# yeeus/GCI

Measured on AMD Instinct MI355X. Metric: aligned Gbases/s through filter+depth pipeline (CHM13, 40x HiFi), higher is better.
Workload: dtype int32

## Files before the change

### gci_amd/csrc/api_ctx.hip

```cpp
#include "gci_ctx.hpp"
#include <stdlib.h>
#include <vector>

int gci_fail(gci_ctx* c, hipError_t e, const char* what)
{
    if (c) c->err = std::string(what) + ": " + hipGetErrorString(e);
    return GCI_E_HIP;
}

int gci_ensure(gci_ctx* ctx, DevBuf& b, size_t bytes)
{
    if (bytes <= b.cap) return GCI_OK;
    if (b.p) { HIPCHK(hipStreamSynchronize(ctx->stream)); HIPCHK(gci_dfree(b.p)); b.p = nullptr; b.cap = 0; }
    size_t want = bytes + bytes / 4 + 256;
    HIPCHK(gci_dmalloc(ctx->device, &b.p, want));
    b.cap = want;
    return GCI_OK;
}

int gci_upload_small(gci_ctx* ctx, void* d_dst, const void* h_src, size_t bytes)
{
    HIPCHK(hipStreamSynchronize(ctx->stream));
    if (bytes > ctx->h_pinned_cap) {
        if (ctx->h_pinned) HIPCHK(hipHostFree(ctx->h_pinned));
        ctx->h_pinned = nullptr;
        ctx->h_pinned_cap = 0;
        size_t want = bytes * 2 + 4096;
        HIPCHK(hipHostMalloc(&ctx->h_pinned, want, hipHostMallocDefault));
        ctx->h_pinned_cap = want;
    }
    memcpy(ctx->h_pinned, h_src, bytes);
    HIPCHK(hipMemcpyAsync(d_dst, ctx->h_pinned, bytes, hipMemcpyHostToDevice, ctx->stream));
    return GCI_OK;
}

extern "C" int gci_abi_version(void) { return GCI_ABI_VERSION; }

extern "C" int gci_ctx_create(int device, void* stream, int own_stream, gci_ctx** out)
{
    if (!out) return GCI_E_INVALID;
    gci_ctx* ctx = new (std::nothrow) gci_ctx();
    if (!ctx) return GCI_E_NOMEM;
    ctx->device = device;
    { const char* fd = getenv("GCI_FORCE_DENSE"); if (fd && fd[0] == '1') ctx->sparse_max = -1; }
    { const char* m = getenv("GCI_JOIN"); ctx->join_mode = m && m[0] == 'c' ? 1 : m && m[0] == 'p' ? 2 : 0; }
    hipError_t e = hipSetDevice(device);
    if (e != hipSuccess) { delete ctx; return GCI_E_HIP; }
    if (!own_stream) { ctx->stream = (hipStream_t)stream; }
    else {
        e = hipStreamCreateWithFlags(&ctx->stream, hipStreamNonBlocking);
        if (e != hipSuccess) { delete ctx; return GCI_E_HIP; }
        ctx->own_stream = true;
    }
    {
        uint32_t lut[TEXT_LUT];
        gci_text_lut_host(lut);
        if (gci_dmalloc(device, &ctx->text_lut.p, sizeof lut) != hipSuccess ||
            hipMemcpy(ctx->text_lut.p, lut, sizeof lut, hipMemcpyHostToDevice) != hipSuccess) {
            gci_ctx_destroy(ctx);
            return GCI_E_HIP;
        }
        ctx->text_lut.cap = sizeof lut;
    }
    *out = ctx;
    return GCI_OK;
}

extern "C" int gci_ctx_destroy(gci_ctx* ctx)
{
    if (!ctx) return GCI_OK;
    (void)hipSetDevice(ctx->device);
    (void)hipStreamSynchronize(ctx->stream);
    DevBuf* bufs[] = {&ctx->d_len, &ctx->d_off, &ctx->d_tile_first, &ctx->tile_cd, &ctx->tile_carry, &ctx->dense_flag, &ctx->dense_list, &ctx->evp_items, &ctx->evp_hist, &ctx->evp_blk, &ctx->d_tile_valid,
                      &ctx->evt_off, &ctx->events, &ctx->blk_a, &ctx->blk_b, &ctx->tile_sum, &ctx->tile_u32,
                      &ctx->tile_u64, &ctx->blk_u64, &ctx->join_table, &ctx->join_last, &ctx->join_hq, &ctx->part_a, &ctx->part_b, &ctx->part_hist, &ctx->part_blk, &ctx->conflict_table, &ctx->win,
                      &ctx->win_tile_first, &ctx->text_lut, &ctx->long_items, &ctx->pg_scan, &ctx->pg_first, &ctx->route_tab, &ctx->deflate_nruns, &ctx->deflate_runs, &ctx->deflate_tab, &ctx->dgz_tiles, &ctx->build_nruns, &ctx->build_runs, &ctx->join_bucket, &ctx->tail_gaps, &ctx->tail_sums, &ctx->class_sums, &ctx->crc_tabs, &ctx->inflate_sym, &ctx->inflate_nsym, &ctx->inflate_wstatus, &ctx->inflate_lists, &ctx->inflate_prof, &ctx->inflate_next, &ctx->inflate_sym2, &ctx->inflate_lists2,
                      &ctx->bg_tile_cnt, &ctx->bg_tile_off, &ctx->bg_blk, &ctx->bg_wtab, &ctx->bg_blk_bytes, &ctx->bg_blk_off, &ctx->bg_blk2, &ctx->hist_chunk_first,
                      &ctx->cover_rec, &ctx->cover_chunk};
    for (DevBuf* b : bufs) if (b->p) (void)gci_dfree(b->p);
    for (DevBuf& b : ctx->paf_pool) if (b.p) (void)gci_dfree(b.p);
    if (ctx->h_pinned) (void)hipHostFree(ctx->h_pinned);
    for (auto* v : {&ctx->prof_live, &ctx->prof_free}) for (auto& e : *v) { (void)hipEventDestroy(e.a); (void)hipEventDestroy(e.b); }
    if (ctx->inflate_stream2) { (void)hipStreamSynchronize(ctx->inflate_stream2); (void)hipStreamDestroy(ctx->inflate_stream2); }
    if (ctx->inflate_ev_in) (void)hipEventDestroy(ctx->inflate_ev_in);
    if (ctx->inflate_ev_out) (void)hipEventDestroy(ctx->inflate_ev_out);
    if (ctx->own_stream) (void)hipStreamDestroy(ctx->stream);
    delete ctx;
    return GCI_OK;
}

extern "C" int gci_sync(gci_ctx* ctx)
{
    if (!ctx) return GCI_E_INVALID;
    HIPCHK(hipStreamSynchronize(ctx->stream));
    return GCI_OK;
}

extern "C" const char* gci_strerror(int s)
{
    switch (s) {
    case GCI_OK: return "ok";
    case GCI_E_INVALID: return "invalid argument";
    case GCI_E_HIP: return "HIP runtime error";
    case GCI_E_NO_NM: return "record without NM tag (reference raises KeyError, GCI.py:163)";
    case GCI_E_ZERO_DIV: return "zero denominator (reference raises ZeroDivisionError, GCI.py:165/292)";
    case GCI_E_BAD_NM_TYPE: return "NM tag is not an integer";
    case GCI_E_NO_END: return "record has no CIGAR: reference_end is None";
    case GCI_E_MALFORMED: return "malformed BAM record";
    case GCI_E_CAPACITY: return "output capacity exceeded";
    case GCI_E_NOMEM: return "out of memory";
    case GCI_E_NO_LAYOUT: return "gci_layout_set() not called";
    default: return "unknown status";
    }
}

extern "C" const char* gci_last_error(gci_ctx* ctx) { return ctx ? ctx->err.c_str() : ""; }

static const char* const PROF_NAMES[GCI_PROF_COUNT] = {
    "k_bam_filter", "k_join_insert", "k_join_fold", "k_evt_count+scatter", "k_scan2", "k_tile_build", "k_gap_mask",
    "k_max2", "k_issue_scan", "k_text_count", "k_text_write", "k_depth_sum", "memset", "k_tile_pass1", "k_tile_dense",
    "k_part1+k_part2 (radix partition of the join)", "k_join_part", "k_pg_measure+scans+k_pg_first (record pages: sizes)", "k_pg_write (record pages)"};

extern "C" int gci_profile_enable(gci_ctx* ctx, int mask)
{
    if (!ctx) return GCI_E_INVALID;
    ctx->prof_mask = mask;
    return GCI_OK;
}

extern "C" int gci_profile_read(gci_ctx* ctx, int kernel_id, double* total_ms, uint64_t* launches, int reset)
{
    if (!ctx || kernel_id < 0 || kernel_id >= GCI_PROF_COUNT) return GCI_E_INVALID;
    HIPCHK(hipStreamSynchronize(ctx->stream));
    for (auto& e : ctx->prof_live) {
        float ms = 0.f;
        if (hipEventElapsedTime(&ms, e.a, e.b) == hipSuccess) { ctx->prof_ms[e.id] += ms; ctx->prof_n[e.id]++; }
        ctx->prof_free.push_back(e);
    }
    ctx->prof_live.clear();
    if (total_ms) *total_ms = ctx->prof_ms[kernel_id];
    if (launches) *launches = ctx->prof_n[kernel_id];
    if (reset) { ctx->prof_ms[kernel_id] = 0; ctx->prof_n[kernel_id] = 0; }
    return GCI_OK;
}

extern "C" const char* gci_profile_name(int kernel_id)
{
    return kernel_id >= 0 && kernel_id < GCI_PROF_COUNT ? PROF_NAMES[kernel_id] : "";
}

extern "C" int gci_malloc(gci_ctx* ctx, size_t bytes, void** d_out)
{
    if (!ctx || !d_out) return GCI_E_INVALID;
    HIPCHK(hipSetDevice(ctx->device));
    HIPCHK(gci_dmalloc(ctx->device, d_out, bytes ? bytes : 16));
    return GCI_OK;
}
extern "C" int gci_free(gci_ctx* ctx, void* p)
{
// ... 87 lines not shown
```

### gci_amd/csrc/gci_ctx.hpp

```cpp
#pragma once
#include <hip/hip_runtime.h>
#include <stdint.h>
#include <stdlib.h>
#include <string.h>
#include <string>
#include <vector>

#include "../../include/gci_hip.h"
#include "gci_common.h"
#include "gci_wave.hpp"

#define TILE GCI_TILE
#define TEXT_LUT 1000
#define BLOCK 256
static_assert(TILE == BLOCK * 16, "a tile is 16 elements per thread");

constexpr int GCI_RUN_MAX = 64;
constexpr uint32_t GCI_RUNS_WALK = 0xFFFFFFFFu;

struct DevBuf {
    void* p = nullptr;
    size_t cap = 0;
};

struct gci_ctx {
    int device = 0;
    hipStream_t stream = nullptr;
    bool own_stream = false;
    std::string err;
    int32_t n_contigs = 0;
    std::vector<int64_t> len, off;
    std::vector<int64_t> tile_first;
    int64_t total = 0, n_tiles = 0;
    DevBuf d_len, d_off, d_tile_first;
    DevBuf tile_cd;
    DevBuf tile_carry;
    DevBuf evt_off;
    DevBuf d_tile_valid;
    DevBuf dense_flag;
    DevBuf dense_list;
    int32_t sparse_max = 62;
    bool join_dirty = false;
    int join_mode = 0;
    uint32_t k1_parity = 0;
    int cd_state = 0;
    int counted_flank = 0;
    bool count_deferred = false;
    DevBuf evp_items, evp_hist, evp_blk;
    DevBuf events;
    DevBuf blk_a, blk_b;
    DevBuf tile_sum;
    DevBuf tile_u32, tile_u64, blk_u64;
    uint32_t build_max_n = 0;
    int build_flank = 0;
    bool build_pending = false, build_text = false;
    bool build_runs_wanted = false;
    DevBuf build_nruns, build_runs;
    const void* build_runs_track = nullptr;
    bool build_runs_armed = false;
    DevBuf join_table, join_last, join_hq;
    DevBuf join_bucket;
    DevBuf part_a, part_b, part_hist, part_blk;
    DevBuf route_tab;
    DevBuf deflate_nruns, deflate_runs;
    DevBuf deflate_tab;
    bool deflate_tab_ready = false;
    DevBuf dgz_tiles;
    uint32_t dgz_members = 0;
    const void* dgz_key = nullptr;
    bool deflate_from_build = false;
    uint32_t deflate_members = 0;
    const void* deflate_key_depth = nullptr;
    const void* deflate_key_elem = nullptr;
    DevBuf conflict_table;
    uint64_t conflict_slots = 0;
    uint32_t conflict_parity = 0;
    DevBuf text_lut;
    DevBuf long_items;
    DevBuf pg_scan, pg_first;
    uint32_t pg_n_rec = 0, pg_page_bytes = 0, pg_n_pages = 0;
    uint32_t pg_cus = 0;
    uint32_t pg_per_cu = 0, pg_per_cu_page_bytes = 0;
    uint64_t pg_blob_off = 0;
    uint64_t pg_blob_bytes = 0;
    std::vector<DevBuf> paf_pool;
    DevBuf crc_tabs;
    bool crc_tabs_ready = false;
    uint32_t inflate_last_n = 0;
    DevBuf inflate_sym, inflate_nsym, inflate_wstatus, inflate_lists, inflate_prof, inflate_next;
    DevBuf inflate_sym2, inflate_lists2;
    int inflate_streams = 1;
    hipStream_t inflate_stream2 = nullptr;
    hipEvent_t inflate_ev_in = nullptr, inflate_ev_out = nullptr;
    DevBuf tail_sums;
    DevBuf class_sums;
    DevBuf tail_gaps;
    std::vector<int64_t> tail_gaps_host;
    DevBuf win, win_tile_first;
    int win_flank = INT32_MIN;
    uint32_t win_n = 0;
    int64_t win_tiles = 0;
    uint64_t win_epoch = 0;
    DevBuf bg_tile_cnt, bg_tile_off, bg_blk, bg_wtab, bg_blk_bytes, bg_blk_off, bg_blk2;
    uint64_t bg_runs_epoch = 0, bg_runs_total = 0;
    const void* bg_runs_track = nullptr;
    const void* bg_text_runs = nullptr;
    const void* bg_text_run0 = nullptr;
    uint32_t bg_text_windows = 0;
    uint64_t bg_text_n_runs = 0, bg_text_total = 0;
    DevBuf hist_chunk_first;
    DevBuf cover_rec, cover_chunk;
    bool cover_valid = false;
    uint32_t cover_n_rec = 0;
    uint64_t cover_n_chunks = 0, cover_n_ivl = 0;
    int cover_count_del = 0;
    const void* cover_stream = nullptr;
    const void* cover_off = nullptr;
    void* h_pinned = nullptr;
    size_t h_pinned_cap = 0;
    int prof_mask = 0;
    struct ProfEv { int id; hipEvent_t a, b; };
    std::vector<ProfEv> prof_live, prof_free;
    double prof_ms[GCI_PROF_COUNT] = {0};
    uint64_t prof_n[GCI_PROF_COUNT] = {0};
};

struct ProfScope {
    gci_ctx* c; gci_ctx::ProfEv ev; bool on;
    ProfScope(gci_ctx* ctx, int kid) : c(ctx), on(false) {
        if (!(ctx->prof_mask & (1 << kid))) return;
        if (!ctx->prof_free.empty()) { ev = ctx->prof_free.back(); ctx->prof_free.pop_back(); }
        else if (hipEventCreate(&ev.a) != hipSuccess || hipEventCreate(&ev.b) != hipSuccess) return;
        ev.id = kid;
        on = hipEventRecord(ev.a, ctx->stream) == hipSuccess;
    }
    ~ProfScope() {
        if (!on) return;
        (void)hipEventRecord(ev.b, c->stream);
        c->prof_live.push_back(ev);
    }
};

int gci_fail(gci_ctx* c, hipError_t e, const char* what);
int gci_ensure(gci_ctx* ctx, DevBuf& b, size_t bytes);
int gci_upload_small(gci_ctx* ctx, void* d_dst, const void* h_src, size_t bytes);

hipError_t gci_dmalloc(int device, void** out, size_t bytes);
hipError_t gci_dfree(void* p);

#define HIPCHK(call)                                      \
    do {                                                  \
        hipError_t _e = (call);                           \
        if (_e != hipSuccess) return gci_fail(ctx, _e, #call); \
    } while (0)
#define LAUNCHCHK(name)                                   \
    do {                                                  \
        hipError_t _e = hipGetLastError();                \
        if (_e != hipSuccess) return gci_fail(ctx, _e, name); \
    } while (0)
#define GCI_TRY(expr)                                     \
    do {                                                  \
        int _r = (expr);                                  \
        if (_r) return _r;                                \
    } while (0)

// ... 302 lines not shown
```

### gci_amd/csrc/k_pages.hip

```cpp
#include "gci_ctx.hpp"

#define PG_MAX_REC GCI_PAGE_MAX_REC
#define PG_MAGIC 0x31504347u
#define PG_EXT 1u
#define PG_OVERSIZE 2u
#define PG_MALFORMED 4u

__device__ __forceinline__ uint32_t a16(uint32_t x) { return (x + 15u) & ~15u; }

__device__ __forceinline__ uint32_t pg_rd16(const uint8_t* p) { return (uint32_t)p[0] | ((uint32_t)p[1] << 8); }
__device__ __forceinline__ uint32_t pg_rd32(const uint8_t* p) { return pg_rd16(p) | (pg_rd16(p + 2) << 16); }

struct PgRec {
    uint32_t kind, size, blob;
    uint32_t lrn, n_cig, aux_len;
    uint64_t aux_off;
    bool short_core;
};

__device__ __forceinline__ PgRec pg_measure(const uint8_t* __restrict__ bam, uint64_t n_bytes, uint64_t off, bool has_seq)
{
    PgRec r;
    r.kind = PG_MALFORMED; r.size = 48; r.blob = 0; r.lrn = r.n_cig = r.aux_len = 0; r.aux_off = 0; r.short_core = false;
    if (off + 36 > n_bytes) { r.short_core = true; return r; }
// ... 140 lines not shown
    const uint32_t inc_c = wave_inclusive<uint32_t>(run_c, lane);
    const unsigned long long inc_b = wave_inclusive<unsigned long long>(run_b, lane);
    if (lane == 63) { wtot[0][wave] = inc_c; wtot[1][wave] = inc_b; }
    __syncthreads();
    uint32_t pre_c = inc_c - run_c, all_c = 0;
    unsigned long long pre_b = inc_b - run_b, all_b = 0;
#pragma unroll
    for (uint32_t w = 0; w < BLOCK / 64; w++) {
        if (w < wave) { pre_c += (uint32_t)wtot[0][w]; pre_b += wtot[1][w]; }
        all_c += (uint32_t)wtot[0][w]; all_b += wtot[1][w];
    }
    const uint32_t base = base0 + t * PER;
#pragma unroll
    for (int i = 0; i < PER; i++) {
        if (base + i <= n_rec) { S_loc[base + i] = pre_c; B_loc[base + i] = pre_b; }
        pre_c += c[i]; pre_b += b[i];
    }
    if (t == 0) { blk_tot[blockIdx.x] = all_c; blk_tot[nb + blockIdx.x] = all_b; }
}

__global__ __launch_bounds__(BLOCK) void k_pg_blk_scan(unsigned long long* __restrict__ blk, uint32_t nb, const uint32_t* __restrict__ S_loc,
                                                       const unsigned long long* __restrict__ B_loc, uint32_t n_rec,
                                                       unsigned long long* __restrict__ tot)
{
    __shared__ unsigned long long wtot[2][BLOCK / 64];
    const uint32_t t = threadIdx.x, lane = t & 63, wave = t >> 6;
    unsigned long long carry_c = 0, carry_b = 0;
    for (uint32_t k0 = 0; k0 < nb; k0 += BLOCK) {
        const uint32_t k = k0 + t;
        const unsigned long long vc = k < nb ? blk[k] : 0ull, vb = k < nb ? blk[nb + k] : 0ull;
        const unsigned long long ic = wave_inclusive<unsigned long long>(vc, lane), ib = wave_inclusive<unsigned long long>(vb, lane);
        if (lane == 63) { wtot[0][wave] = ic; wtot[1][wave] = ib; }
        __syncthreads();
        unsigned long long pc = carry_c + ic - vc, pb = carry_b + ib - vb;
#pragma unroll
        for (uint32_t w = 0; w < BLOCK / 64; w++) {
            if (w < wave) { pc += wtot[0][w]; pb += wtot[1][w]; }
            carry_c += wtot[0][w]; carry_b += wtot[1][w];
        }
        if (k < nb) { blk[k] = pc; blk[nb + k] = pb; }
        __syncthreads();
    }
    if (t == 0) {
        const PgSums s = {S_loc, B_loc, blk, nb};
        tot[0] = pg_S(s, n_rec - 1); tot[1] = pg_S(s, n_rec); tot[2] = pg_B(s, n_rec);
    }
}

struct PgWin { const uint8_t* lds; const uint8_t* lo; const uint8_t* hi; };

__device__ __forceinline__ bool pg_in_win(const PgWin& W, const uint8_t* p, uint32_t len) { return p >= W.lo && p + len <= W.hi; }

__device__ __forceinline__ uint4 pg_piece(const uint8_t* __restrict__ bam, uint64_t n_bytes, const PgWin& W, bool in_win, uint64_t src,
                                          uint32_t len, uint32_t roff)
{
    uint32_t w[4] = {0u, 0u, 0u, 0u};
    if (roff >= len) return make_uint4(0, 0, 0, 0);
    if (in_win) {
        const uint8_t* q = W.lds + (uint32_t)(bam + src - W.lo) + roff;
        const uint32_t left = len - roff;
#pragma unroll
        for (int d = 0; d < 4; d++) {
            w[d] = pg_lds32(q + 4 * d);
            if (left < 4u * d + 4u) w[d] = left > 4u * d ? w[d] & ((1u << (8u * (left - 4u * d))) - 1u) : 0u;
        }
    } else {
#pragma unroll
        for (int d = 0; d < 4; d++) if (roff + 4u * d < len) w[d] = pg_src_dword(bam, n_bytes, src, len, roff / 4u + d);
    }
    return make_uint4(w[0], w[1], w[2], w[3]);
}

#ifndef PG_BLOCK
#define PG_BLOCK BLOCK
#endif
#ifndef PG_WIN_DIV
#define PG_WIN_DIV 1
#endif
#define PG_WIN_SLACK 16u
#define PG_WIN_REGS (8 / PG_WIN_DIV)
static_assert(GCI_PAGE_MAX_BYTES / PG_WIN_DIV <= PG_WIN_REGS * PG_BLOCK * 16, "a thread holds its share of a whole window in registers");
static inline __host__ __device__ uint32_t pg_win_cap(uint32_t page_bytes) { return (page_bytes / PG_WIN_DIV) & ~15u; }

__device__ __forceinline__ PgWin pg_win_of(const uint8_t* lds, const uint8_t* bam, const uint8_t* end, uint64_t off0, uint64_t span_end, uint32_t cap)
{
    PgWin W;
    W.lds = lds; W.lo = W.hi = bam;
    if (off0 < span_end) {
        const uint8_t* p0 = bam + off0;
        const uint8_t* lo = p0 - ((uintptr_t)p0 & 15u);
        if (lo < bam) lo += 16;
        const uint8_t* last = bam + span_end + 15;
        const uint8_t* hi = last - ((uintptr_t)last & 15u);
        if (hi > end) hi = end - ((uintptr_t)end & 15u);
        if (hi > lo) { W.lo = lo; W.hi = (uint64_t)(hi - lo) < cap ? hi : lo + cap; }
    }
    return W;
}
__device__ __forceinline__ void pg_win_load(const PgWin& W, uint32_t t, uint4 v[PG_WIN_REGS])
{
    const uint32_t pieces = (uint32_t)(W.hi - W.lo) / 16u;
#pragma unroll
    for (int u = 0; u < PG_WIN_REGS; u++) {
        const uint32_t i = u * PG_BLOCK + t;
        v[u] = i < pieces ? reinterpret_cast<const uint4*>(W.lo)[i] : make_uint4(0, 0, 0, 0);
    }
}
__device__ __forceinline__ void pg_win_store(uint8_t* win, const PgWin& W, uint32_t t, const uint4 v[PG_WIN_REGS])
{
    const uint32_t pieces = (uint32_t)(W.hi - W.lo) / 16u;
#pragma unroll
    for (int u = 0; u < PG_WIN_REGS; u++) {
        const uint32_t i = u * PG_BLOCK + t;
        if (i < pieces) reinterpret_cast<uint4*>(win)[i] = v[u];
    }
}

struct PgPage { uint32_t first, cnt; uint64_t off0, span_end; };
__device__ __forceinline__ PgPage pg_page_of(const PgArgs& A, uint32_t k)
{
    PgPage p;
    p.first = A.page_first[k]; p.cnt = A.page_first[k + 1] - p.first;
    p.off0 = A.page_off[k];
    p.span_end = A.page_off[k + 1];
    if (p.span_end > A.n_bytes) p.span_end = A.n_bytes;
    return p;
}
struct PgMine { uint64_t off; unsigned long long S, S0, S_end; };
__device__ __forceinline__ PgMine pg_mine_of(const PgArgs& A, const PgPage& p, uint32_t t)
{
    PgMine m;
    m.off = 0; m.S = 0;
    if (t < p.cnt && t < PG_META_MAX) { m.off = A.rec_off[p.first + t]; m.S = pg_S(A.sums, p.first + t); }
    m.S0 = p.cnt ? pg_S(A.sums, p.first) : 0ull;
    m.S_end = p.cnt ? pg_S(A.sums, p.first + p.cnt) : 0ull;
    return m;
}

#ifndef PG_PERSIST
#define PG_PERSIST 1
#endif
#ifndef PG_WAVES
#define PG_WAVES 4
#endif
__global__ __launch_bounds__(PG_BLOCK) __attribute__((amdgpu_waves_per_eu(PG_WAVES, PG_WAVES))) void k_pg_write(const PgArgs A)
{
    extern __shared__ __attribute__((aligned(16))) uint8_t win[];
    __shared__ uint16_t s_blob_rec[GCI_PAGE_MAX_BYTES / 48];
    __shared__ uint32_t s_n_blob, s_take, s_sparse;
    __shared__ PgMeta s_meta[PG_META_MAX];
    __shared__ __attribute__((aligned(16))) uint32_t s_core[PG_META_MAX][12];
    __shared__ uint8_t s_map[GCI_PAGE_MAX_BYTES / 16];
    __shared__ __attribute__((aligned(16))) uint8_t s_head[16 + ((2 * ((GCI_PAGE_MAX_BYTES - 16) / 50) + 15) & ~15)];
    const uint32_t t = threadIdx.x, G = gridDim.x;
    const uint32_t P = A.page_bytes;
    const uint32_t win_cap = pg_win_cap(P);
    const uint8_t* end = A.bam + A.n_bytes;
    const PgPage none = {0u, 0u, 0ull, 0ull};

    uint32_t k = blockIdx.x;
    PgPage p_next = pg_page_of(A, k);
    PgPage p_after = k + G < A.n_pages ? pg_page_of(A, k + G) : none;
    PgWin W_next = pg_win_of(win, A.bam, end, p_next.off0, p_next.span_end, win_cap);
    uint4 v[PG_WIN_REGS];
    pg_win_load(W_next, t, v);
    PgMine m_next = pg_mine_of(A, p_next, t);

    for (; k < A.n_pages; k += G) {
        const PgPage pg = p_next;
        const PgMine mine = m_next;
        const PgWin W0 = W_next;
        const uint32_t first = pg.first, cnt = pg.cnt;
        const unsigned long long S0 = mine.S0;
        const uint32_t rec0 = 16u + a16(2u * cnt);
        const uint32_t used = cnt ? rec0 + (uint32_t)(mine.S_end - S0) - 2u * cnt : 16u;
        uint4* const g = reinterpret_cast<uint4*>(A.out + (uint64_t)k * P);
        pg_win_store(win, W0, t, v);
        if (t < sizeof(s_head) / 16) reinterpret_cast<uint4*>(s_head)[t] = make_uint4(0, 0, 0, 0);
        if (t == 0) {
            s_n_blob = 0;
            uint32_t* h = reinterpret_cast<uint32_t*>(s_head);
            h[0] = cnt; h[1] = first; h[2] = used; h[3] = PG_MAGIC;
        }
        p_next = p_after;
        if (k + G < A.n_pages) {
            W_next = pg_win_of(win, A.bam, end, p_next.off0, p_next.span_end, win_cap);
            pg_win_load(W_next, t, v);
            m_next = pg_mine_of(A, p_next, t);
        }
        p_after = (uint64_t)k + 2ull * G < A.n_pages ? pg_page_of(A, k + 2 * G) : none;

        if (cnt == 0) __syncthreads();
        for (uint32_t m0 = 0; m0 < cnt;) {
            const uint32_t mc = cnt - m0 < PG_META_MAX ? cnt - m0 : PG_META_MAX;
            uint64_t off0 = pg.off0, off = mine.off;
            unsigned long long Si = mine.S;
            PgWin W = W0;
            if (m0) {
                off0 = A.rec_off[first + m0];
                W = pg_win_of(win, A.bam, end, off0, pg.span_end, win_cap);
                uint4 w[PG_WIN_REGS];
                pg_win_load(W, t, w);
                if (t < mc) { off = A.rec_off[first + m0 + t]; Si = pg_S(A.sums, first + m0 + t); }
                pg_win_store(win, W, t, w);
            }
            if (t == 0) { s_take = mc; s_sparse = 0u; }
            __syncthreads();
            uint32_t my_blob = 0;
            if (t < mc) {
                const uint32_t j = m0 + t, i = first + j;
                uint32_t core[12];
                PgRec r;
                bool core_in = false;
                if (off + 36 > A.n_bytes) {
#pragma unroll
                    for (int d = 0; d < 9; d++) core[d] = 0u;
                    r.kind = PG_MALFORMED; r.size = 48; r.blob = 0; r.lrn = r.n_cig = r.aux_len = 0; r.aux_off = 0; r.short_core = true;
                    core_in = true;
                } else {
                    const uint8_t* p = A.bam + off;
                    core_in = pg_in_win(W, p, 36);
                    if (core_in) {
#pragma unroll
                        for (int d = 0; d < 9; d++) core[d] = pg_lds32(win + (uint32_t)(p - W.lo) + 4 * d);
                    } else {
                        pg_core_gather(A.bam, A.n_bytes, off, core);
                    }
                    r = pg_classify(core, A.n_bytes, off, A.has_seq != 0);
                }
                const bool copied = r.kind == 0 || r.kind == PG_EXT;
                const uint32_t cig_len = r.kind == 0 ? 4u * r.n_cig : r.n_cig ? 4u : 0u;
                uint32_t in = 0;
                if (copied) {
                    if (pg_in_win(W, A.bam + off + 36, r.lrn)) in |= PG_IN_NAME;
                    if (pg_in_win(W, A.bam + off + 36 + r.lrn, cig_len)) in |= PG_IN_CIGAR;
                    if (pg_in_win(W, A.bam + r.aux_off, r.aux_len)) in |= PG_IN_AUX;
                }
                if (t == 0) { if (!core_in || (copied && in != (PG_IN_NAME | PG_IN_CIGAR | PG_IN_AUX))) s_sparse = 1u; }
                else if (off >= off0 && A.bam + off + 36 > W.hi) atomicMin(&s_take, t);
                const uint32_t at = rec0 + (uint32_t)(Si - S0) - 2u * j;
                const uint64_t blob_at = r.blob ? A.blob_off + pg_B(A.sums, i) : 0ull;
                my_blob = r.blob;
                *reinterpret_cast<uint16_t*>(s_head + 16 + 2 * j) = (uint16_t)(at >> 4);
                core[0] = r.size;
                core[3] = (core[3] & 0xFFFFu) | (r.kind << 16);
                core[6] = r.aux_len; core[7] = (uint32_t)blob_at; core[8] = (uint32_t)(blob_at >> 32);
                if (r.kind == PG_MALFORMED) core[6] = core[7] = core[8] = 0u;
                const uint4 nm = copied ? pg_piece(A.bam, A.n_bytes, W, (in & PG_IN_NAME) != 0, off + 36, r.lrn, 0) : make_uint4(0, 0, 0, 0);
                core[9] = nm.x; core[10] = nm.y; core[11] = nm.z;
#pragma unroll
                for (int d = 0; d < 12; d += 4) *reinterpret_cast<uint4*>(&s_core[t][d]) = make_uint4(core[d], core[d + 1], core[d + 2], core[d + 3]);
                for (uint32_t q = 0; q < r.size / 16u; q++) s_map[(at >> 4) + q] = (uint8_t)t;
                PgMeta mt;
                mt.off = off; mt.aux_off = r.aux_off; mt.lrn = (uint8_t)r.lrn; mt.n_cig = (uint16_t)r.n_cig;
                mt.aux_len = (uint16_t)(r.aux_len <= PG_MAX_REC ? r.aux_len : 0u);
                mt.at = (uint16_t)at; mt.kind = (uint8_t)(r.kind | in);
                s_meta[t] = mt;
            }
            __syncthreads();
            const uint32_t take = __builtin_amdgcn_readfirstlane(s_sparse ? mc : s_take);
            if (t < take && my_blob) s_blob_rec[atomicAdd(&s_n_blob, 1u)] = (uint16_t)(m0 + t);
            const uint32_t piece_lo = s_meta[0].at >> 4;
            const uint32_t piece_hi = m0 + take == cnt ? used >> 4 : take < mc ? s_meta[take].at >> 4
                                                                               : (rec0 + (uint32_t)(pg_S(A.sums, first + m0 + take) - S0) - 2u * (m0 + take)) >> 4;
            for (uint32_t piece = piece_lo + t; piece < piece_hi; piece += PG_BLOCK) {
                const uint32_t jj = s_map[piece];
                const PgMeta mt = s_meta[jj];
                const uint32_t q = 16u * piece - mt.at, kind = mt.kind & 0xFu;
                uint4 o;
                if (q < 48u) o = *reinterpret_cast<const uint4*>(&s_core[jj][q / 4u]);
                else {
                    const uint32_t c = a16(36u + mt.lrn), c2 = c + (kind == 0 ? a16(4u * mt.n_cig) : 16u);
                    if (q < c) o = pg_piece(A.bam, A.n_bytes, W, (mt.kind & PG_IN_NAME) != 0, mt.off + 36, mt.lrn, q - 36u);
                    else if (q < c2) o = pg_piece(A.bam, A.n_bytes, W, (mt.kind & PG_IN_CIGAR) != 0, mt.off + 36 + mt.lrn,
                                                  kind == 0 ? 4u * mt.n_cig : mt.n_cig ? 4u : 0u, q - c);
                    else o = pg_piece(A.bam, A.n_bytes, W, (mt.kind & PG_IN_AUX) != 0, mt.aux_off, mt.aux_len, q - c2);
                }
                g[piece] = o;
            }
            __syncthreads();
            m0 += take;
        }
        for (uint32_t piece = t; piece < rec0 / 16u; piece += PG_BLOCK) g[piece] = reinterpret_cast<const uint4*>(s_head)[piece];
        for (uint32_t piece = (used >> 4) + t; piece < P / 16u; piece += PG_BLOCK) g[piece] = make_uint4(0, 0, 0, 0);
        const uint32_t n_blob = s_n_blob;
        for (uint32_t b = 0; b < n_blob; b++) {
            const uint32_t i = first + s_blob_rec[b];
            const uint64_t off = A.rec_off[i];
            const PgRec r = pg_measure(A.bam, A.n_bytes, off, A.has_seq != 0);
            if (!r.blob) continue;
            uint32_t* o = reinterpret_cast<uint32_t*>(A.out + A.blob_off + pg_B(A.sums, i));
            if (r.kind == PG_EXT) {
                for (uint32_t d = t; d < r.blob / 4; d += PG_BLOCK)
                    o[d] = d < r.n_cig ? pg_src_dword(A.bam, A.n_bytes, off + 36 + r.lrn, 4 * r.n_cig, d) : 0u;
            } else {
                const uint32_t head = 36 + r.lrn + 4 * r.n_cig, total = head + r.aux_len;
                for (uint32_t d = t; d < r.blob / 4; d += PG_BLOCK) {
                    uint32_t w = 0;
                    const uint32_t b0 = 4 * d;
                    if (b0 + 4 <= head) w = pg_src_dword(A.bam, A.n_bytes, off, head, d);
                    else if (b0 >= head) { if (b0 < total) w = pg_src_dword(A.bam, A.n_bytes, r.aux_off + (b0 - head), total - b0, 0); }
                    else {
                        for (uint32_t x0 = 0; x0 < 4 && b0 + x0 < total; x0++) {
                            const uint32_t x = b0 + x0;
                            w |= (uint32_t)(x < head ? A.bam[off + x] : A.bam[r.aux_off + (x - head)]) << (8 * x0);
                        }
                    }
                    if (d == 0) w = total - 4;
                    o[d] = w;
                }
            }
        }
        __syncthreads();
    }
}

static inline PgSums pg_sums_of(gci_ctx* ctx, uint32_t n_rec)
{
    PgSums s;
    s.nb = n_rec / TILE + 1;
    s.B_loc = (const unsigned long long*)ctx->pg_scan.p + 3;
    s.blk = s.B_loc + (size_t)n_rec + 1;
    s.S_loc = (const uint32_t*)(s.blk + 2 * (size_t)s.nb);
    return s;
}
static inline int pg_sums_ensure(gci_ctx* ctx, uint32_t n_rec)
{
    return gci_ensure(ctx, ctx->pg_scan, (3 + 2 * ((size_t)n_rec / TILE + 1)) * 8 + ((size_t)n_rec + 1) * (8 + 4));
}

extern "C" int gci_bam_pages_size(gci_ctx* ctx, const uint8_t* d_stream, uint64_t n_bytes, const uint64_t* d_rec_off, uint32_t n_rec,
                                  int has_seq, uint32_t page_bytes, uint64_t* h_out)
{
    if (!ctx || !h_out || (n_rec && (!d_stream || !d_rec_off))) return GCI_E_INVALID;
    if (page_bytes < 8192 || page_bytes > GCI_PAGE_MAX_BYTES || (page_bytes & 4095u)) return GCI_E_INVALID;
    h_out[0] = h_out[1] = h_out[2] = 0;
    ctx->pg_n_rec = n_rec; ctx->pg_page_bytes = page_bytes; ctx->pg_n_pages = 0; ctx->pg_blob_off = 0; ctx->pg_blob_bytes = 0;
    if (n_rec == 0) { h_out[1] = 16; return GCI_OK; }
    const uint32_t Q = page_bytes - PG_MAX_REC - 48;
    GCI_TRY(pg_sums_ensure(ctx, n_rec));
    const PgSums sums = pg_sums_of(ctx, n_rec);
    unsigned long long* tot = (unsigned long long*)ctx->pg_scan.p;
    {
        ProfScope _ps(ctx, GCI_PROF_PAGES_SIZE);
        hipLaunchKernelGGL(k_pg_measure, dim3(sums.nb), dim3(BLOCK), 0, ctx->stream, d_stream, n_bytes, d_rec_off, n_rec, has_seq,
                           (uint32_t*)sums.S_loc, (unsigned long long*)sums.B_loc, (unsigned long long*)sums.blk, sums.nb);
        LAUNCHCHK("k_pg_measure");
        hipLaunchKernelGGL(k_pg_blk_scan, dim3(1), dim3(BLOCK), 0, ctx->stream, (unsigned long long*)sums.blk, sums.nb, sums.S_loc, sums.B_loc,
                           n_rec, tot);
        LAUNCHCHK("k_pg_blk_scan");
    }
    unsigned long long tail[3];
    HIPCHK(hipMemcpyAsync(tail, tot, 24, hipMemcpyDeviceToHost, ctx->stream));
    HIPCHK(hipStreamSynchronize(ctx->stream));
    const unsigned long long b_total = tail[2];
    const uint64_t n_pages = tail[0] / Q + 1;
    if (n_pages > 0xFFFFFFF0ull) return GCI_E_INVALID;
    GCI_TRY(gci_ensure(ctx, ctx->pg_first, (size_t)(n_pages + 1) * (8 + 4)));
    uint64_t* page_off = (uint64_t*)ctx->pg_first.p;
    hipLaunchKernelGGL(k_pg_first, dim3((uint32_t)((n_pages + 1 + BLOCK - 1) / BLOCK)), dim3(BLOCK), 0, ctx->stream, sums, n_rec,
                       (uint32_t)n_pages, Q, d_rec_off, n_bytes, (uint32_t*)(page_off + n_pages + 1), page_off);
    LAUNCHCHK("k_pg_first");
    ctx->pg_n_pages = (uint32_t)n_pages;
    ctx->pg_blob_off = n_pages * page_bytes;
    ctx->pg_blob_bytes = b_total;
    h_out[0] = n_pages;
    h_out[1] = n_pages * page_bytes + b_total + 16;
    h_out[2] = ctx->pg_blob_off;
    return GCI_OK;
}

extern "C" int gci_bam_pages_write(gci_ctx* ctx, const uint8_t* d_stream, uint64_t n_bytes, const uint64_t* d_rec_off, uint32_t n_rec,
                                   int has_seq, uint8_t* d_out, uint64_t cap)
{
    if (!ctx || !d_out || (n_rec && (!d_stream || !d_rec_off))) return GCI_E_INVALID;
    if (n_rec != ctx->pg_n_rec) return GCI_E_INVALID;
    if (n_rec == 0) { HIPCHK(hipMemsetAsync(d_out, 0, cap < 16 ? cap : 16, ctx->stream)); return GCI_OK; }
    PgArgs A;
    A.bam = d_stream; A.n_bytes = n_bytes; A.rec_off = d_rec_off; A.n_rec = n_rec; A.has_seq = has_seq;
    A.sums = pg_sums_of(ctx, n_rec); A.page_off = (const uint64_t*)ctx->pg_first.p; A.page_first = (const uint32_t*)(A.page_off + ctx->pg_n_pages + 1);
    A.n_pages = ctx->pg_n_pages; A.page_bytes = ctx->pg_page_bytes;
    A.blob_off = ctx->pg_blob_off; A.out = d_out;
    const uint64_t need = ctx->pg_blob_off + ctx->pg_blob_bytes + 16;
    if (cap < need) return GCI_E_CAPACITY;
    const uint32_t lds = pg_win_cap(ctx->pg_page_bytes) + PG_WIN_SLACK;
    if (!ctx->pg_cus) {
        int cus = 0;
        HIPCHK(hipDeviceGetAttribute(&cus, hipDeviceAttributeMultiprocessorCount, ctx->device));
        ctx->pg_cus = cus > 0 ? (uint32_t)cus : 256u;
    }
    if (ctx->pg_per_cu_page_bytes != ctx->pg_page_bytes) {
        int per_cu = 0;
        HIPCHK(hipOccupancyMaxActiveBlocksPerMultiprocessor(&per_cu, k_pg_write, PG_BLOCK, lds));
        ctx->pg_per_cu = per_cu > 0 ? (uint32_t)per_cu : 1u;
        ctx->pg_per_cu_page_bytes = ctx->pg_page_bytes;
    }
    const uint32_t resident = ctx->pg_cus * ctx->pg_per_cu;
    {
        ProfScope _ps(ctx, GCI_PROF_PAGES_WRITE);
        hipLaunchKernelGGL(k_pg_write, dim3(PG_PERSIST && resident < ctx->pg_n_pages ? resident : ctx->pg_n_pages), dim3(PG_BLOCK), lds, ctx->stream, A);
        LAUNCHCHK("k_pg_write");
    }
    HIPCHK(hipMemsetAsync(d_out + need - 16, 0, 16, ctx->stream));
    return GCI_OK;
}
```

Measured before the change: 22910.

## Add lean fast-path page writer with fallback list for hard pages

When sequences are absent, a new templated kernel writes each page from a register-staged window using a descriptor-driven LDS gather and nontemporal buffer stores. Pages it cannot handle are appended to a worklist that the original general writer then processes. The trailing guard memset is folded into the writer kernel, and an env var can cap the grid size. This is meant to cut per-page cost for the common case, at the price of an extra kernel launch and duplicated logic.

```diff
diff --git a/gci_amd/csrc/api_ctx.hip b/gci_amd/csrc/api_ctx.hip
--- a/gci_amd/csrc/api_ctx.hip
+++ b/gci_amd/csrc/api_ctx.hip
@@ -44,6 +44,7 @@
     ctx->device = device;
     { const char* fd = getenv("GCI_FORCE_DENSE"); if (fd && fd[0] == '1') ctx->sparse_max = -1; }
     { const char* m = getenv("GCI_JOIN"); ctx->join_mode = m && m[0] == 'c' ? 1 : m && m[0] == 'p' ? 2 : 0; }
+    { const char* g = getenv("GCI_PAGES_GRID"); const long n = g ? atol(g) : 0; ctx->pg_grid_cap = n > 0 && n < (1 << 20) ? (uint32_t)n : 0u; }
     hipError_t e = hipSetDevice(device);
     if (e != hipSuccess) { delete ctx; return GCI_E_HIP; }
     if (!own_stream) { ctx->stream = (hipStream_t)stream; }
@@ -74,7 +75,7 @@
     DevBuf* bufs[] = {&ctx->d_len, &ctx->d_off, &ctx->d_tile_first, &ctx->tile_cd, &ctx->tile_carry, &ctx->dense_flag, &ctx->dense_list, &ctx->evp_items, &ctx->evp_hist, &ctx->evp_blk, &ctx->d_tile_valid,
                       &ctx->evt_off, &ctx->events, &ctx->blk_a, &ctx->blk_b, &ctx->tile_sum, &ctx->tile_u32,
                       &ctx->tile_u64, &ctx->blk_u64, &ctx->join_table, &ctx->join_last, &ctx->join_hq, &ctx->part_a, &ctx->part_b, &ctx->part_hist, &ctx->part_blk, &ctx->conflict_table, &ctx->win,
-                      &ctx->win_tile_first, &ctx->text_lut, &ctx->long_items, &ctx->pg_scan, &ctx->pg_first, &ctx->route_tab, &ctx->deflate_nruns, &ctx->deflate_runs, &ctx->deflate_tab, &ctx->dgz_tiles, &ctx->build_nruns, &ctx->build_runs, &ctx->join_bucket, &ctx->tail_gaps, &ctx->tail_sums, &ctx->class_sums, &ctx->crc_tabs, &ctx->inflate_sym, &ctx->inflate_nsym, &ctx->inflate_wstatus, &ctx->inflate_lists, &ctx->inflate_prof, &ctx->inflate_next, &ctx->inflate_sym2, &ctx->inflate_lists2,
+                      &ctx->win_tile_first, &ctx->text_lut, &ctx->long_items, &ctx->pg_scan, &ctx->pg_first, &ctx->pg_list, &ctx->route_tab, &ctx->deflate_nruns, &ctx->deflate_runs, &ctx->deflate_tab, &ctx->dgz_tiles, &ctx->build_nruns, &ctx->build_runs, &ctx->join_bucket, &ctx->tail_gaps, &ctx->tail_sums, &ctx->class_sums, &ctx->crc_tabs, &ctx->inflate_sym, &ctx->inflate_nsym, &ctx->inflate_wstatus, &ctx->inflate_lists, &ctx->inflate_prof, &ctx->inflate_next, &ctx->inflate_sym2, &ctx->inflate_lists2,
                       &ctx->bg_tile_cnt, &ctx->bg_tile_off, &ctx->bg_blk, &ctx->bg_wtab, &ctx->bg_blk_bytes, &ctx->bg_blk_off, &ctx->bg_blk2, &ctx->hist_chunk_first,
                       &ctx->cover_rec, &ctx->cover_chunk};
     for (DevBuf* b : bufs) if (b->p) (void)gci_dfree(b->p);
diff --git a/gci_amd/csrc/gci_ctx.hpp b/gci_amd/csrc/gci_ctx.hpp
--- a/gci_amd/csrc/gci_ctx.hpp
+++ b/gci_amd/csrc/gci_ctx.hpp
@@ -81,6 +81,10 @@
     uint32_t pg_n_rec = 0, pg_page_bytes = 0, pg_n_pages = 0;
     uint32_t pg_cus = 0;
     uint32_t pg_per_cu = 0, pg_per_cu_page_bytes = 0;
+    uint32_t pg_lean_per_cu = 0, pg_lean_page_bytes = 0;
+    uint32_t pg_grid_cap = 0;
+    DevBuf pg_list;
+    uint32_t pg_parity = 0;
     uint64_t pg_blob_off = 0;
     uint64_t pg_blob_bytes = 0;
     std::vector<DevBuf> paf_pool;
diff --git a/gci_amd/csrc/k_pages.hip b/gci_amd/csrc/k_pages.hip
--- a/gci_amd/csrc/k_pages.hip
+++ b/gci_amd/csrc/k_pages.hip
@@ -246,7 +246,8 @@
 static_assert(GCI_PAGE_MAX_BYTES / PG_WIN_DIV <= PG_WIN_REGS * PG_BLOCK * 16, "a thread holds its share of a whole window in registers");
 static inline __host__ __device__ uint32_t pg_win_cap(uint32_t page_bytes) { return (page_bytes / PG_WIN_DIV) & ~15u; }
 
-__device__ __forceinline__ PgWin pg_win_of(const uint8_t* lds, const uint8_t* bam, const uint8_t* end, uint64_t off0, uint64_t span_end, uint32_t cap)
+__device__ __forceinline__ PgWin pg_win_of(const uint8_t* lds, const uint8_t* bam, const uint8_t* end, uint64_t off0, uint64_t span_end, uint32_t cap,
+                                           bool whole_only = false)
 {
     PgWin W;
     W.lds = lds; W.lo = W.hi = bam;
@@ -257,7 +258,7 @@
         const uint8_t* last = bam + span_end + 15;
         const uint8_t* hi = last - ((uintptr_t)last & 15u);
         if (hi > end) hi = end - ((uintptr_t)end & 15u);
-        if (hi > lo) { W.lo = lo; W.hi = (uint64_t)(hi - lo) < cap ? hi : lo + cap; }
+        if (hi > lo && !(whole_only && (uint64_t)(hi - lo) > cap)) { W.lo = lo; W.hi = (uint64_t)(hi - lo) < cap ? hi : lo + cap; }
     }
     return W;
 }
@@ -307,7 +308,8 @@
 #ifndef PG_WAVES
 #define PG_WAVES 4
 #endif
-__global__ __launch_bounds__(PG_BLOCK) __attribute__((amdgpu_waves_per_eu(PG_WAVES, PG_WAVES))) void k_pg_write(const PgArgs A)
+__global__ __launch_bounds__(PG_BLOCK) __attribute__((amdgpu_waves_per_eu(PG_WAVES, PG_WAVES))) void k_pg_write(const PgArgs A, const uint32_t* __restrict__ n_listed,
+                                                                                                                const uint32_t* __restrict__ listed, uint8_t* __restrict__ guard)
 {
     extern __shared__ __attribute__((aligned(16))) uint8_t win[];
     __shared__ uint16_t s_blob_rec[GCI_PAGE_MAX_BYTES / 48];
@@ -322,15 +324,21 @@
     const uint8_t* end = A.bam + A.n_bytes;
     const PgPage none = {0u, 0u, 0ull, 0ull};
 
-    uint32_t k = blockIdx.x;
+    if (blockIdx.x == 0 && t < 16) guard[t] = 0;
+    const uint32_t n_items = listed ? *n_listed : A.n_pages;
+    uint32_t it = blockIdx.x;
+    if (it >= n_items) return;
+    uint32_t k = listed ? listed[it] : it;
+    uint32_t k_after = it + G < n_items ? (listed ? listed[it + G] : it + G) : 0u;
     PgPage p_next = pg_page_of(A, k);
-    PgPage p_after = k + G < A.n_pages ? pg_page_of(A, k + G) : none;
-    PgWin W_next = pg_win_of(win, A.bam, end, p_next.off0, p_next.span_end, win_cap);
+    PgPage p_after = it + G < n_items ? pg_page_of(A, k_after) : none;
+    PgWin W_next = pg_win_of(win, A.bam, end, p_next.off0, p_next.span_end, win_cap, true);
     uint4 v[PG_WIN_REGS];
     pg_win_load(W_next, t, v);
     PgMine m_next = pg_mine_of(A, p_next, t);
 
-    for (; k < A.n_pages; k += G) {
+    uint32_t k_next = 0u;
+    for (; it < n_items; it += G, k = k_next) {
         const PgPage pg = p_next;
         const PgMine mine = m_next;
         const PgWin W0 = W_next;
@@ -347,12 +355,15 @@
             h[0] = cnt; h[1] = first; h[2] = used; h[3] = PG_MAGIC;
         }
         p_next = p_after;
-        if (k + G < A.n_pages) {
-            W_next = pg_win_of(win, A.bam, end, p_next.off0, p_next.span_end, win_cap);
+        if (it + G < n_items) {
+            W_next = pg_win_of(win, A.bam, end, p_next.off0, p_next.span_end, win_cap, true);
             pg_win_load(W_next, t, v);
             m_next = pg_mine_of(A, p_next, t);
         }
-        p_after = (uint64_t)k + 2ull * G < A.n_pages ? pg_page_of(A, k + 2 * G) : none;
+        const bool two_on = (uint64_t)it + 2ull * G < n_items;
+        k_next = k_after;
+        k_after = two_on ? (listed ? listed[it + 2 * G] : it + 2 * G) : 0u;
+        p_after = two_on ? pg_page_of(A, k_after) : none;
 
         if (cnt == 0) __syncthreads();
         for (uint32_t m0 = 0; m0 < cnt;) {
@@ -479,6 +490,187 @@
     }
 }
 
+struct PglWin { const uint8_t* lo; uint32_t pieces; };
+__device__ __forceinline__ PglWin pgl_win_of(const PgArgs& A, const PgPage& p, uint32_t cap)
+{
+    PglWin W;
+    W.lo = A.bam; W.pieces = 0;
+    if (p.cnt == 0 || p.cnt > PG_META_MAX || p.off0 >= p.span_end) return W;
+    const uint8_t* p0 = A.bam + p.off0;
+    const uint8_t* lo = p0 - ((uintptr_t)p0 & 15u);
+    const uint8_t* last = A.bam + p.span_end + 15;
+    const uint8_t* hi = last - ((uintptr_t)last & 15u);
+    if (lo < A.bam || hi > A.bam + A.n_bytes || (uint64_t)(hi - lo) > cap) return W;
+    W.lo = lo; W.pieces = (uint32_t)(hi - lo) / 16u;
+    return W;
+}
+
+struct PglTab { uint32_t first, first1; uint64_t off0, off1; };
+__device__ __forceinline__ uint32_t pgl_rfl(uint32_t x) { return __builtin_amdgcn_readfirstlane(x); }
+__device__ __forceinline__ uint64_t pgl_rfl(uint64_t x) { return pgl_rfl((uint32_t)x) | ((uint64_t)pgl_rfl((uint32_t)(x >> 32)) << 32); }
+__device__ __forceinline__ PglTab pgl_tab_of(const PgArgs& A, uint32_t k, uint32_t z)
+{
+    PglTab r;
+    r.first = A.page_first[k + z]; r.first1 = A.page_first[k + 1 + z]; r.off0 = A.page_off[k + z]; r.off1 = A.page_off[k + 1 + z];
+    return r;
+}
+__device__ __forceinline__ PgPage pgl_page_of(const PgArgs& A, const PglTab& r)
+{
+    PgPage p;
+    p.first = pgl_rfl(r.first); p.cnt = pgl_rfl(r.first1) - p.first; p.off0 = pgl_rfl(r.off0); p.span_end = pgl_rfl(r.off1);
+    if (p.span_end > A.n_bytes) p.span_end = A.n_bytes;
+    return p;
+}
+struct PglSum { uint32_t loc, blk; };
+__device__ __forceinline__ PglSum pgl_sum_of(const PgSums& s, uint32_t i)
+{
+    PglSum r;
+    r.loc = s.S_loc[i]; r.blk = reinterpret_cast<const uint32_t*>(s.blk)[2u * (i / TILE)];
+    return r;
+}
+__device__ __forceinline__ uint32_t pgl_diff(const PglSum& a, const PglSum& b) { return (a.loc + a.blk) - (b.loc + b.blk); }
+__device__ __forceinline__ PglSum pgl_rfl(const PglSum& a) { PglSum r; r.loc = pgl_rfl(a.loc); r.blk = pgl_rfl(a.blk); return r; }
+struct PglMine { uint64_t off; PglSum S, S0, S_end; };
+__device__ __forceinline__ PglMine pgl_mine_of(const PgArgs& A, const PgPage& p, uint32_t t, uint32_t z)
+{
+    PglMine m;
+    m.off = 0; m.S.loc = 0; m.S.blk = 0;
+    if (t < p.cnt && t < PG_META_MAX) { m.off = A.rec_off[p.first + t]; m.S = pgl_sum_of(A.sums, p.first + t); }
+    m.S0 = pgl_sum_of(A.sums, p.first + z);
+    m.S_end = pgl_sum_of(A.sums, p.first + p.cnt + z);
+    return m;
+}
+
+typedef uint32_t pgl_u32x4 __attribute__((ext_vector_type(4)));
+__device__ __forceinline__ uint4 pgl_load16(const uint4* p)
+{
+    const pgl_u32x4 x = __builtin_nontemporal_load(reinterpret_cast<const pgl_u32x4*>(p));
+    return make_uint4(x[0], x[1], x[2], x[3]);
+}
+#define PGL_STORE_NT 2
+
+template <int NP>
+__global__ __launch_bounds__(PG_BLOCK) __attribute__((amdgpu_waves_per_eu(NP > 6 ? 3 : PG_WAVES, NP > 6 ? 3 : PG_WAVES))) void k_pg_lean(const PgArgs A, uint32_t* __restrict__ n_listed,
+                                                                                                               uint32_t* __restrict__ listed, uint32_t* __restrict__ n_listed_next)
+{
+    constexpr uint32_t P = NP * 16u * PG_BLOCK;
+    constexpr uint32_t HEAD = P + PG_WIN_SLACK, HEAD_BYTES = 16u + 2u * PG_META_MAX, CORE = HEAD + HEAD_BYTES;
+    __shared__ __attribute__((aligned(16))) uint8_t lds[CORE + 48u * PG_META_MAX];
+    __shared__ uint32_t s_desc[P / 16];
+    __shared__ __attribute__((aligned(16))) uint32_t s_mask[17][4];
+    __shared__ uint32_t s_rel[PG_META_MAX];
+    __shared__ uint32_t s_bad;
+    const uint32_t t = threadIdx.x, G = gridDim.x;
+    if (blockIdx.x == 0 && t == 0) *n_listed_next = 0u;
+    if (t < 17u) {
+#pragma unroll
+        for (int d = 0; d < 4; d++) s_mask[t][d] = t >= 4u * d + 4u ? ~0u : t > 4u * d ? (1u << (8u * (t - 4u * d))) - 1u : 0u;
+    }
+
+    uint32_t k = blockIdx.x;
+    const PglTab no_tab = {0u, 0u, 0ull, 0ull};
+    uint32_t z;
+    asm("v_mov_b32 %0, 0" : "=v"(z));
+    PgPage p_next = pg_page_of(A, k);
+    PglTab tab_after = k + G < A.n_pages ? pgl_tab_of(A, k + G, z) : no_tab;
+    PglWin W_next = pgl_win_of(A, p_next, P);
+    uint4 v[NP];
+#pragma unroll
+    for (int u = 0; u < NP; u++) {
+        const uint32_t i = u * PG_BLOCK + t;
+        v[u] = i < W_next.pieces ? pgl_load16(reinterpret_cast<const uint4*>(W_next.lo) + i) : make_uint4(0, 0, 0, 0);
+    }
+    PglMine m_next = pgl_mine_of(A, p_next, t, z);
+    __builtin_amdgcn_s_waitcnt(0x0F70);
+
+    for (; k < A.n_pages; k += G) {
+        const PgPage pg = p_next;
+        PglMine mine = m_next;
+        mine.S0 = pgl_rfl(mine.S0); mine.S_end = pgl_rfl(mine.S_end);
+        const PglWin W = W_next;
+        const uint32_t cnt = pg.cnt;
+        const uint32_t rec0 = 16u + a16(2u * cnt);
+        uint32_t used = cnt ? rec0 + pgl_diff(mine.S_end, mine.S0) - 2u * cnt : 16u;
+        if (used > P) used = P;
+#pragma unroll
+        for (int u = 0; u < NP; u++) {
+            const uint32_t i = u * PG_BLOCK + t;
+            if (i < W.pieces) reinterpret_cast<uint4*>(lds)[i] = v[u];
+        }
+        const uint64_t rel64 = (uint64_t)(A.bam + mine.off - W.lo);
+        const uint32_t rel = rel64 < 16ull * W.pieces ? (uint32_t)rel64 : ~0u;
+        if (t < PG_META_MAX) s_rel[t] = rel;
+        if (t < HEAD_BYTES / 16u) reinterpret_cast<uint4*>(lds + HEAD)[t] = t ? make_uint4(0, 0, 0, 0) : make_uint4(cnt, pg.first, used, PG_MAGIC);
+        if (t == 0) s_bad = W.pieces ? 0u : 1u;
+        __syncthreads();
+        p_next = pgl_page_of(A, tab_after);
+        if (k + G < A.n_pages) {
+            W_next = pgl_win_of(A, p_next, P);
+#pragma unroll
+            for (int u = 0; u < NP; u++) {
+                const uint32_t i = u * PG_BLOCK + t;
+                v[u] = i < W_next.pieces ? pgl_load16(reinterpret_cast<const uint4*>(W_next.lo) + i) : make_uint4(0, 0, 0, 0);
+            }
+            m_next = pgl_mine_of(A, p_next, t, z);
+        }
+        tab_after = (uint64_t)k + 2ull * G < A.n_pages ? pgl_tab_of(A, k + 2 * G, z) : no_tab;
+        if (W.pieces && t < cnt) {
+            const uint32_t win_bytes = 16u * W.pieces;
+            bool good = rel != ~0u && rel + 36u <= win_bytes && (t == 0 || s_rel[t - 1] < rel);
+            if (good) {
+                uint32_t core[12];
+#pragma unroll
+                for (int d = 0; d < 12; d++) core[d] = pg_lds32(lds + rel + 4 * d);
+                const PgRec r = pg_classify(core, A.n_bytes, mine.off, false);
+                const uint32_t at = rec0 + pgl_diff(mine.S, mine.S0) - 2u * t;
+                const uint32_t src_len = 36u + r.lrn + 4u * r.n_cig + r.aux_len;
+                good = r.kind == 0 && rel + src_len <= win_bytes && (at & 15u) == 0 && at >= rec0 && at + r.size <= used;
+                if (good) {
+                    *reinterpret_cast<uint16_t*>(lds + HEAD + 16 + 2 * t) = (uint16_t)(at >> 4);
+                    core[0] = r.size;
+                    core[3] &= 0xFFFFu;
+                    core[6] = r.aux_len; core[7] = 0u; core[8] = 0u;
+#pragma unroll
+                    for (int d = 0; d < 3; d++)
+                        core[9 + d] = r.lrn >= 4u * d + 4u ? core[9 + d] : r.lrn > 4u * d ? core[9 + d] & ((1u << (8u * (r.lrn - 4u * d))) - 1u) : 0u;
+#pragma unroll
+                    for (int d = 0; d < 12; d += 4) *reinterpret_cast<uint4*>(lds + CORE + 48u * t + 4u * d) = make_uint4(core[d], core[d + 1], core[d + 2], core[d + 3]);
+                    uint32_t* d = s_desc + (at >> 4);
+                    const uint32_t name_end = 36u + r.lrn, cig = 4u * r.n_cig, c = a16(name_end);
+                    d[0] = (CORE + 48u * t) | (16u << 16); d[1] = (CORE + 48u * t + 16u) | (16u << 16); d[2] = (CORE + 48u * t + 32u) | (16u << 16);
+                    d += 3;
+                    for (uint32_t b = 48u; b < c; b += 16u) *d++ = (rel + b) | ((name_end - b < 16u ? name_end - b : 16u) << 16);
+                    for (uint32_t b = 0; b < cig; b += 16u) *d++ = (rel + name_end + b) | ((cig - b < 16u ? cig - b : 16u) << 16);
+                    for (uint32_t b = 0; b < r.aux_len; b += 16u) *d++ = (rel + name_end + cig + b) | ((r.aux_len - b < 16u ? r.aux_len - b : 16u) << 16);
+                }
+            }
+            if (!good) s_bad = 1u;
+        }
+#pragma unroll
+        for (int u = 0; u < NP; u++) {
+            const uint32_t piece = u * PG_BLOCK + t;
+            if (piece < rec0 / 16u) s_desc[piece] = (HEAD + 16u * piece) | (16u << 16);
+            else if (piece >= used / 16u) s_desc[piece] = 0u;
+        }
+        __syncthreads();
+        const bool lean = __builtin_amdgcn_readfirstlane(s_bad) == 0u;
+        const __amdgpu_buffer_rsrc_t page = __builtin_amdgcn_make_buffer_rsrc(A.out + (uint64_t)k * P, 0, lean ? P : 0u, 0x00020000);
+#pragma unroll
+        for (int u = 0; u < NP; u++) {
+            const uint32_t piece = u * PG_BLOCK + t;
+            const uint32_t desc = lean ? s_desc[piece] : 0u;
+            const uint32_t src = desc & 0xFFFFu;
+            const uint4 m = *reinterpret_cast<const uint4*>(s_mask[desc >> 16 < 16u ? desc >> 16 : 16u]);
+            pgl_u32x4 o;
+            o[0] = pg_lds32(lds + src) & m.x; o[1] = pg_lds32(lds + src + 4) & m.y;
+            o[2] = pg_lds32(lds + src + 8) & m.z; o[3] = pg_lds32(lds + src + 12) & m.w;
+            __builtin_amdgcn_raw_buffer_store_b128(o, page, 16u * piece, 0, PGL_STORE_NT);
+        }
+        if (!lean && t == 0) listed[atomicAdd(n_listed, 1u)] = k;
+        __syncthreads();
+    }
+}
+
 static inline PgSums pg_sums_of(gci_ctx* ctx, uint32_t n_rec)
 {
     PgSums s;
@@ -534,6 +726,21 @@
     return GCI_OK;
 }
 
+typedef void (*pg_lean_fn)(const PgArgs, uint32_t*, uint32_t*, uint32_t*);
+static inline pg_lean_fn pg_lean_of(uint32_t page_bytes)
+{
+    static_assert(GCI_PAGE_MAX_BYTES == 8 * 16 * PG_BLOCK, "k_pg_lean is instantiated for 2 .. 8 pieces per thread");
+    switch (page_bytes / (16u * PG_BLOCK)) {
+    case 2: return k_pg_lean<2>;
+    case 3: return k_pg_lean<3>;
+    case 4: return k_pg_lean<4>;
+    case 5: return k_pg_lean<5>;
+    case 6: return k_pg_lean<6>;
+    case 7: return k_pg_lean<7>;
+    default: return k_pg_lean<8>;
+    }
+}
+
 extern "C" int gci_bam_pages_write(gci_ctx* ctx, const uint8_t* d_stream, uint64_t n_bytes, const uint64_t* d_rec_off, uint32_t n_rec,
                                    int has_seq, uint8_t* d_out, uint64_t cap)
 {
@@ -559,12 +766,35 @@
         ctx->pg_per_cu = per_cu > 0 ? (uint32_t)per_cu : 1u;
         ctx->pg_per_cu_page_bytes = ctx->pg_page_bytes;
     }
-    const uint32_t resident = ctx->pg_cus * ctx->pg_per_cu;
-    {
-        ProfScope _ps(ctx, GCI_PROF_PAGES_WRITE);
-        hipLaunchKernelGGL(k_pg_write, dim3(PG_PERSIST && resident < ctx->pg_n_pages ? resident : ctx->pg_n_pages), dim3(PG_BLOCK), lds, ctx->stream, A);
+    const auto grid_of = [&](uint32_t per_cu) {
+        uint32_t g = ctx->pg_cus * per_cu;
+        if (!PG_PERSIST || g > ctx->pg_n_pages) g = ctx->pg_n_pages;
+        return ctx->pg_grid_cap && g > ctx->pg_grid_cap ? ctx->pg_grid_cap : g;
+    };
+    uint8_t* const guard = d_out + need - 16;
+    ProfScope _ps(ctx, GCI_PROF_PAGES_WRITE);
+    if (has_seq) {
+        hipLaunchKernelGGL(k_pg_write, dim3(grid_of(ctx->pg_per_cu)), dim3(PG_BLOCK), lds, ctx->stream, A, (const uint32_t*)nullptr, (const uint32_t*)nullptr, guard);
         LAUNCHCHK("k_pg_write");
-    }
-    HIPCHK(hipMemsetAsync(d_out + need - 16, 0, 16, ctx->stream));
+        return GCI_OK;
+    }
+    const size_t cap_before = ctx->pg_list.cap;
+    GCI_TRY(gci_ensure(ctx, ctx->pg_list, 16 + 4 * (size_t)ctx->pg_n_pages));
+    if (ctx->pg_list.cap != cap_before) { HIPCHK(hipMemsetAsync(ctx->pg_list.p, 0, 16, ctx->stream)); ctx->pg_parity = 0; }
+    uint32_t* const counters = (uint32_t*)ctx->pg_list.p;
+    uint32_t* const listed = counters + 4;
+    const uint32_t par = ctx->pg_parity;
+    const pg_lean_fn lean = pg_lean_of(ctx->pg_page_bytes);
+    if (ctx->pg_lean_page_bytes != ctx->pg_page_bytes) {
+        int per_cu = 0;
+        HIPCHK(hipOccupancyMaxActiveBlocksPerMultiprocessor(&per_cu, lean, PG_BLOCK, 0));
+        ctx->pg_lean_per_cu = per_cu > 0 ? (uint32_t)per_cu : 1u;
+        ctx->pg_lean_page_bytes = ctx->pg_page_bytes;
+    }
+    ctx->pg_parity ^= 1u;
+    hipLaunchKernelGGL(lean, dim3(grid_of(ctx->pg_lean_per_cu)), dim3(PG_BLOCK), 0, ctx->stream, A, counters + par, listed, counters + (par ^ 1u));
+    LAUNCHCHK("k_pg_lean");
+    hipLaunchKernelGGL(k_pg_write, dim3(grid_of(ctx->pg_per_cu)), dim3(PG_BLOCK), lds, ctx->stream, A, (const uint32_t*)(counters + par), (const uint32_t*)listed, guard);
+    LAUNCHCHK("k_pg_write");
     return GCI_OK;
 }
```

Result: faster. 24320, median of 6 (+6.2%).
